# roatienza/efficientspeech

Hardware: AMD Instinct MI355X
Metric: mel-frames/sec (whole node), full Phoneme2Mel forward (higher is better)
Workload: dtype f32 (weight GEMMs: fp32 operands split into 2 f16 pieces (22 significand bits, weights pre-scaled 2^8), 3 f16-MFMA products, fp32 accumulate)

## Files before the change

efficientspeech_amd/csrc/chain16.h:

```cpp
#pragma once
#include "esmi_dev.h"
#include "wave_chain.h"

namespace esmi {
namespace c16 {

typedef unsigned u32x2 __attribute__((ext_vector_type(2)));

__device__ __forceinline__ float row_sum4(float v) {
    v += swap16_f(v);
    v += swap32_f(v);
    return v;
}
__device__ __forceinline__ float row_max4(float v) {
    v = fmaxf(v, swap16_f(v));
    v = fmaxf(v, swap32_f(v));
    return v;
}

__device__ __forceinline__ f32x4 mma(const u32x4& w1, const u32x4& w2, const f16x2p& a, f32x4 c) {
    c = mfma16_f16(w1, a.h2, c);
    c = mfma16_f16(w2, a.h1, c);
    c = mfma16_f16(w1, a.h1, c);
    return c;
// ... 17 lines not shown
    }
}

template <int N>
struct WFrags { u32x4 w1[N], w2[N]; };
template <int NT16, int NTW, int N>
__device__ __forceinline__ void wfrags_load(WFrags<N>& f, int at, const float* W0, int lw, int G) {
#pragma unroll
    for (int nt = 0; nt < NT16; ++nt) {
        const float* wp = W0 + ((4 * G) * NTW + (nt >> 1)) * 256 + 64 * (nt & 1) + lw;
        f.w1[at + nt] = *reinterpret_cast<const u32x4*>(wp);
        f.w2[at + nt] = *reinterpret_cast<const u32x4*>(wp + NTW * 256);
    }
}
template <int N>
__device__ __forceinline__ void mma_all(f32x4 (&acc)[N], const WFrags<N>& f, const f16x2p& a) {
#pragma unroll
    for (int n = 0; n < N; ++n) acc[n] = mfma16_f16(f.w1[n], a.h2, acc[n]);
#pragma unroll
    for (int n = 0; n < N; ++n) acc[n] = mfma16_f16(f.w2[n], a.h1, acc[n]);
#pragma unroll
    for (int n = 0; n < N; ++n) acc[n] = mfma16_f16(f.w1[n], a.h1, acc[n]);
}
template <int NT16, int NTW, int KS, typename BOp>
__device__ __forceinline__ void gemm_pf(f32x4 (&acc)[NT16], const float* W0, int lw, int G0, BOp bop) {
    WFrags<NT16> f[KS];
#pragma unroll
    for (int ks = 0; ks < KS; ++ks) wfrags_load<NT16, NTW, NT16>(f[ks], 0, W0, lw, G0 + ks);
    sched_fence();
#pragma unroll
    for (int ks = 0; ks < KS; ++ks) mma_all<NT16>(acc, f[ks], bop(ks));
}

__device__ __forceinline__ f16x2p planes_load(const unsigned* rowp, int ks, int chalf) {
    f16x2p a;
    a.h1 = *reinterpret_cast<const u32x4*>(rowp + 16 * ks);
    a.h2 = *reinterpret_cast<const u32x4*>(rowp + 16 * ks + chalf);
    return a;
}
__device__ __forceinline__ int wpos(int lane) { const int g = lane >> 4; return 4 * (g & 1) + 2 * (g >> 1); }
__device__ __forceinline__ void planes_store(unsigned* rowp, int nt, int chalf, const f32x4& v) {
    unsigned h1a, h2a, h1b, h2b;
    split_f16_pair(v[0], v[1], h1a, h2a);
    split_f16_pair(v[2], v[3], h1b, h2b);
    *reinterpret_cast<u32x2*>(rowp + 8 * nt) = u32x2{h1a, h1b};
    *reinterpret_cast<u32x2*>(rowp + 8 * nt + chalf) = u32x2{h2a, h2b};
}
__device__ __forceinline__ unsigned gl_lane(int lane) { const int g = lane >> 4; return (unsigned)((16 * (g >> 1) + 4 * (g & 1)) * 4); }
__device__ __forceinline__ f16x2p global_bop(BufRsrc r, unsigned off, int ks) {
    const f32x4 x0 = buf_ld4(r, off + 128u * ks), x1 = buf_ld4(r, off + 128u * ks + 32u);
    return split_f16x2(x0, x1);
}

template <int NT16>
__device__ __forceinline__ void layernorm(f32x4 (&v)[NT16], const f32x4 (&g)[NT16], const f32x4 (&b)[NT16], float eps = 1e-5f) {
    const float inv_c = 1.0f / (float)(16 * NT16);
    float s = 0.0f;
#pragma unroll
    for (int nt = 0; nt < NT16; ++nt) s += (v[nt][0] + v[nt][1]) + (v[nt][2] + v[nt][3]);
    const float mean = row_sum4(s) * inv_c;
    float q = 0.0f;
#pragma unroll
    for (int nt = 0; nt < NT16; ++nt) {
#pragma unroll
        for (int e = 0; e < 4; ++e) {
            v[nt][e] -= mean;
            q = fmaf(v[nt][e], v[nt][e], q);
        }
    }
    const float rstd = rsqrt_fast_f32(row_sum4(q) * inv_c + eps);
#pragma unroll
    for (int nt = 0; nt < NT16; ++nt) {
#pragma unroll
        for (int e = 0; e < 4; ++e) v[nt][e] = fmaf(v[nt][e] * rstd, g[nt][e], b[nt][e]);
    }
}

__device__ __forceinline__ void dma_frags(const float* gsrc, float* ldst, int nfrag, int w, int nw, int lane, int rot = 0) {
    rot %= nfrag;
    for (int f = w; f < nfrag; f += nw) {
        int fr = f + rot;
        fr = fr >= nfrag ? fr - nfrag : fr;
        lds_dma16(gsrc + fr * 256 + 4 * lane, ldst + fr * 256, lane);
    }
}

__device__ __forceinline__ f32x4 ld4_lds(const float* p) { return *reinterpret_cast<const f32x4*>(p); }
__device__ __forceinline__ f32x4 fmaf4(const f32x4& v, float s, const f32x4& b) {
    f32x4 o;
#pragma unroll
    for (int e = 0; e < 4; ++e) o[e] = fmaf(v[e], s, b[e]);
    return o;
}
__device__ __forceinline__ f32x4 relu4(const f32x4& v) {
    f32x4 o;
#pragma unroll
    for (int e = 0; e < 4; ++e) o[e] = fmaxf(v[e], 0.0f);
    return o;
}

}
}
```

efficientspeech_amd/csrc/enc_block16.h:

```cpp
#pragma once
#include "chain16.h"
#include "enc_attn_ffn.h"

namespace esmi {

struct B016Lds {
    static constexpr int C = 32, LD = C + 4, NK = 128, LDX = NK + 4;
    static constexpr int xP = 0;
    static constexpr int xT = xP + 128 * LD;
    static constexpr int y1P = xT + C * LDX;
    static constexpr int priv = y1P + 130 * LD;
    static constexpr int priv_sz = 2 * 16 * LD;
    static constexpr int par = priv + 8 * priv_sz;
    static constexpr int wts = par + 512;
    static constexpr int total = wts + 24 * 256;
};
static_assert(B016Lds::total * 4 <= 160 * 1024, "enc_b0_16: LDS");
enum { B0_PROJB = 0, B0_LN1G = 32, B0_LN1B = 64, B0_FFNB = 96, B0_FFNB0 = 128, B0_FFNB2 = 160, B0_MLP2B = 192, B0_LN2G = 224, B0_LN2B = 256 };

template <int NKT>
__device__ __forceinline__ void enc_b0_16_body(const EncAttnFfnP& p) {
    using namespace c16;
    typedef B016Lds M;
    constexpr int C = M::C, LD = M::LD, LDX = M::LDX;
    ESMI_DYN_LDS(lds);
    ESMI_CT_INIT(0);
    ESMI_CT();
    const int nw = (int)(blockDim.x >> 6), w = uniform_i(wave_id());
    const int lane = lane_id(), i = lane & 15, g = lane >> 4;
    const int b = (int)blockIdx.x, rot = b;
    const int pos = 16 * w + i;
    unsigned* const ldu = reinterpret_cast<unsigned*>(lds);
    unsigned* const xP = ldu + M::xP;
    unsigned* const xT = ldu + M::xT;
    unsigned* const y1P = ldu + M::y1P;
    float* const xf = lds + M::priv + w * M::priv_sz;
    unsigned* const qP = ldu + M::priv + w * M::priv_sz + 16 * LD;
    float* const par = lds + M::par;
    float* const wM = lds + M::wts, * const wO = wM + 4 * 256, * const wF = wO + 4 * 256, * const w2 = wF + 12 * 256;
    const int wp = wpos(lane), lw1 = wlane(lane, 1);
    const f32x4 z4 = zero4();
    const int* idb = p.m.ids + (long)b * p.m.n_in;
    int id[3];
#pragma unroll
    for (int j = 0; j < 3; ++j) {
        const int ti = pos + j - 1;
        const bool ok = ti >= 0 && ti < p.m.n_in;
        const int v = idb[ok ? ti : 0];
        id[j] = !ok ? -1 : ((v < 0 || v >= p.m.vocab) ? 0 : v);
    }
    dma_frags(p.m.qkv_w, wM, 4, w, nw, lane, rot);
    dma_frags(p.proj_w, wO, 4, w, nw, lane, rot);
    dma_frags(p.ffn_w, wF, 12, w, nw, lane, rot);
    dma_frags(p.mlp2_w, w2, 4, w, nw, lane, rot);
    {
        const int v8 = lane >> 3, c8 = 4 * (lane & 7);
        auto pick8 = [&](const float* a0, const float* a1, const float* a2, const float* a3, const float* a4, const float* a5, const float* a6,
                         const float* a7) __attribute__((always_inline)) {
            const float* lo = v8 & 1 ? (v8 & 2 ? a3 : a1) : (v8 & 2 ? a2 : a0);
            const float* hi = v8 & 1 ? (v8 & 2 ? a7 : a5) : (v8 & 2 ? a6 : a4);
            return (v8 & 4 ? hi : lo) + c8;
        };
        if (w == 0 % nw) lds_dma16(pick8(p.proj_b, p.ln1_g, p.ln1_b, p.ffn_b, p.ffn_b0, p.ffn_b2, p.mlp2_b, p.ln2_g), par, lane);
        if (w == 1 % nw) lds_dma16(p.ln2_b + c8, par + B0_LN2B, lane);
    }
    if (w == 0 && lane < LD) {
        y1P[lane] = 0u;
        y1P[(16 * nw + 1) * LD + lane] = 0u;
    }
    if (nw < NKT) {
        for (int e = (int)threadIdx.x; e < C * LDX; e += (int)blockDim.x) xT[e] = 0u;
        for (int e = (int)threadIdx.x + 16 * nw * LD; e < 16 * NKT * LD; e += (int)blockDim.x) xP[e] = 0u;
        wg_sync_lds();
    }
// ... 125 lines not shown
        for (int nt = 0; nt < 2; ++nt) {
            const f32x4 pb = ld4_lds(par + B0_PROJB + 16 * nt + 4 * g);
            gg[nt] = ld4_lds(par + B0_LN1G + 16 * nt + 4 * g);
            bb[nt] = ld4_lds(par + B0_LN1B + 16 * nt + 4 * g);
            y[nt] = fmaf4(y[nt], kF16WScaleInv, pb) + xacc[nt];
        }
        layernorm<2>(y, gg, bb);
#pragma unroll
        for (int nt = 0; nt < 2; ++nt) {
            if (rz || rout) y[nt] = z4;
            planes_store(y1P + (1 + pos) * LD + wp, nt, C / 2, y[nt]);
        }
    }
    ESMI_CT();
    wg_sync_lds();
    ESMI_CT();
    {
        f32x4 m[2] = {z4, z4};
        WFrags<2> ff[3];
        f16x2p fa[3];
#pragma unroll
        for (int j = 0; j < 3; ++j) {
            fa[j] = planes_load(y1P + (pos + j) * LD + 4 * g, 0, C / 2);
            wfrags_load<2, 1, 2>(ff[j], 0, wF + 4 * j * 256, lw1, 0);
        }
        sched_fence();
#pragma unroll
        for (int j = 0; j < 3; ++j) mma_all<2>(m, ff[j], fa[j]);
#pragma unroll
        for (int nt = 0; nt < 2; ++nt) {
            const f32x4 cb = ld4_lds(par + B0_FFNB + 16 * nt + 4 * g), cb0 = ld4_lds(par + B0_FFNB0 + 16 * nt + 4 * g),
                        cb2 = ld4_lds(par + B0_FFNB2 + 16 * nt + 4 * g);
            f32x4 v;
#pragma unroll
            for (int e = 0; e < 4; ++e) {
                const float bias = cb[e] - (pos == 0 ? cb0[e] : 0.0f) - (pos == p.N - 1 ? cb2[e] : 0.0f);
                v[e] = gelu_fast_f32(fmaf(m[nt][e], kF16WScaleInv, bias));
            }
            planes_store(qP + i * LD + wp, nt, C / 2, v);
        }
        lds_wave_sync();
        f32x4 z[2] = {z4, z4};
        const unsigned* rowp = qP + i * LD + 4 * g;
        gemm_pf<2, 1, 1>(z, w2, lw1, 0, [&](int) __attribute__((always_inline)) { return planes_load(rowp, 0, C / 2); });
        f32x4 gg[2], bb[2];
#pragma unroll
        for (int nt = 0; nt < 2; ++nt) {
            const f32x4 b2 = ld4_lds(par + B0_MLP2B + 16 * nt + 4 * g);
            gg[nt] = ld4_lds(par + B0_LN2G + 16 * nt + 4 * g);
            bb[nt] = ld4_lds(par + B0_LN2B + 16 * nt + 4 * g);
            z[nt] = fmaf4(z[nt], kF16WScaleInv, b2) + y[nt];
        }
        layernorm<2>(z, gg, bb);
        const BufRsrc r_out = make_rsrc(p.out + (long)b * p.N * C, (long)p.N * C * 4);
        const unsigned off = rout ? kBufOOB : (unsigned)(pos * C * 4);
#pragma unroll
        for (int nt = 0; nt < 2; ++nt) buf_st4(r_out, off + (unsigned)((16 * nt + 4 * g) * 4), rz ? z4 : z[nt]);
    }
    ESMI_CT();
}

template <int NKT>
__global__ __launch_bounds__(64 * 8, 2) void enc_b0_16_kernel(const EncAttnFfnP p) {
    enc_b0_16_body<NKT>(p);
}

struct B116Lds {
    static constexpr int C = 64, LD = C + 4, CIN = 32, NK = 64, LDX = NK + 4, LDC = 2 * C + 4;
    static constexpr int r1 = 0;
    static constexpr int r2 = r1 + 66 * LD;
    static constexpr int r3 = r2 + 64 * LD;
    static constexpr int r3_sz = 8 * 16 * LD;
    static constexpr int stats = r3 + r3_sz;
    static constexpr int par = stats + 256;
    static constexpr int wY = par + 768;
    static constexpr int wX = wY + 48 * 256;
    static constexpr int total = wX + 32 * 256;
};
static_assert(64 * B116Lds::LDC <= B116Lds::r3_sz && B116Lds::total * 4 <= 160 * 1024, "enc_b1_16: LDS");
enum { B1_PROJB = 0, B1_LN1G = 64, B1_LN1B = 128, B1_FFNB = 192, B1_FFNB0 = 256, B1_FFNB2 = 320, B1_MLP2B = 384, B1_LN2G = 448, B1_LN2B = 512 };

__device__ __forceinline__ void layernorm_pair16(f32x4 (&v)[2], const f32x4 (&gg)[2], const f32x4 (&bb)[2], float* st, int c, int i, int g,
                                                 float eps = 1e-5f) {
    using namespace c16;
    float s = (v[0][0] + v[0][1]) + (v[0][2] + v[0][3]) + ((v[1][0] + v[1][1]) + (v[1][2] + v[1][3]));
    const float mean_l = row_sum4(s) * (1.0f / 32.0f);
    float q = 0.0f;
#pragma unroll
    for (int nt = 0; nt < 2; ++nt) {
#pragma unroll
        for (int e = 0; e < 4; ++e) {
            const float d = v[nt][e] - mean_l;
            q = fmaf(d, d, q);
        }
    }
    const float m2_l = row_sum4(q);
    if (g == 0) *reinterpret_cast<f32x2*>(st + (c * 16 + i) * 2) = f32x2{mean_l, m2_l};
    wg_sync_lds();
    const f32x2 o = *reinterpret_cast<const f32x2*>(st + ((c ^ 1) * 16 + i) * 2);
    const float ma = c == 0 ? mean_l : o[0], mb = c == 0 ? o[0] : mean_l;
    const float qa = c == 0 ? m2_l : o[1], qb = c == 0 ? o[1] : m2_l;
    const float mean = 0.5f * (ma + mb);
    const float d = mb - ma;
    const float m2 = (qa + qb) + d * d * 16.0f;
    const float rstd = rsqrt_fast_f32(m2 * (1.0f / 64.0f) + eps);
#pragma unroll
    for (int nt = 0; nt < 2; ++nt) {
#pragma unroll
        for (int e = 0; e < 4; ++e) v[nt][e] = fmaf((v[nt][e] - mean) * rstd, gg[nt][e], bb[nt][e]);
    }
}

__device__ __forceinline__ void enc_b1_16_body(const EncAttnFfnP& p) {
    using namespace c16;
    typedef B116Lds M;
    constexpr int C = M::C, LD = M::LD, LDX = M::LDX, LDC = M::LDC, CIN = M::CIN, NKT = 4;
    ESMI_DYN_LDS(lds);
    ESMI_CT_INIT(1);
    ESMI_CT();
    const int nw = (int)(blockDim.x >> 6), w = uniform_i(wave_id());
    const int nrt = nw >> 1, rt = w >> 1, c = w & 1;
    const int lane = lane_id(), i = lane & 15, g = lane >> 4;
    const int b = (int)blockIdx.x, rot = b;
    const int pos = 16 * rt + i;
    unsigned* const ldu = reinterpret_cast<unsigned*>(lds);
    unsigned* const xP = ldu + M::r1;
    unsigned* const y1P = ldu + M::r1;
    unsigned* const xT = ldu + M::r2;
    unsigned* const hidP = ldu + M::r2;
    float* const xf = lds + M::r3 + w * (16 * LD);
    unsigned* const qP = ldu + M::r3 + w * (16 * LD);
    unsigned* const ctxP = ldu + M::r3;
    float* const st = lds + M::stats + rt * 64;
    float* const par = lds + M::par;
    float* const wY = lds + M::wY, * const wX = lds + M::wX;
    const int wp = wpos(lane), lw2 = wlane(lane, 2), lw4 = wlane(lane, 4);
    const f32x4 z4 = zero4();
    const bool rout = pos >= p.N;
    const BufRsrc r_in = make_rsrc(p.m.x_in + (long)b * p.m.n_in * CIN, (long)p.m.n_in * CIN * 4);
    const f16x2p a_in = global_bop(r_in, rout ? kBufOOB : (unsigned)(2 * pos * CIN * 4) + gl_lane(lane), 0);
    dma_frags(p.m.merge_w, wY, 8, w, nw, lane, rot);
    dma_frags(p.m.qkv_w, wY + 8 * 256, 32, w, nw, lane, rot);
    dma_frags(p.proj_w, wX, 32, w, nw, lane, rot);
    {
        const int v4 = lane >> 4, c4 = 4 * (lane & 15);
        auto pick4 = [&](const float* a0, const float* a1, const float* a2, const float* a3) __attribute__((always_inline)) {
            return (v4 & 2 ? (v4 & 1 ? a3 : a2) : (v4 & 1 ? a1 : a0)) + c4;
        };
        if (w == 0 % nw) lds_dma16(pick4(p.proj_b, p.ln1_g, p.ln1_b, p.ffn_b), par, lane);
        if (w == 1 % nw) lds_dma16(pick4(p.ffn_b0, p.ffn_b2, p.mlp2_b, p.ln2_g), par + 256, lane);
        if (w == 2 % nw) lds_dma16(p.ln2_b + c4, par + 512, lane);
    }
    if (nrt < NKT) {
        for (int e = (int)threadIdx.x; e < C * LDX; e += (int)blockDim.x) xT[e] = 0u;
        for (int e = (int)threadIdx.x + 16 * nrt * LD; e < 16 * NKT * LD; e += (int)blockDim.x) xP[e] = 0u;
        wg_sync_lds();
    }
    unsigned mb = 0;
    {
        const BufRsrc r_mask = make_rsrc(p.mask ? p.mask + (long)b * p.mask_len : nullptr, p.mask_len);
        for (int q = 0; q < p.mask_pool; ++q) {
            const int idx = pos * p.mask_pool + q;
            mb |= buf_ld_u8(r_mask, (unsigned)idx) | (unsigned)(p.mask && idx >= p.mask_len);
        }
    }
    const bool rz = !rout && mb != 0;
    wait_vm0();
    wg_sync_lds();
    ESMI_CT();
    f32x4 xh[2] = {z4, z4};
    gemm_pf<2, 2, 1>(xh, wY + c * 256, lw2, 0, [&](int) __attribute__((always_inline)) { return a_in; });
#pragma unroll
    for (int nt = 0; nt < 2; ++nt) {
        xh[nt] = rout ? z4 : xh[nt] * kF16WScaleInv;
        planes_store(xP + pos * LD + wp, 2 * c + nt, C / 2, xh[nt]);
        *reinterpret_cast<f32x4*>(xf + i * (CIN + 4) + 16 * nt + 4 * g) = xh[nt];
    }
    lds_wave_sync();
#pragma unroll
    for (int ct = 0; ct < 2; ++ct) {
        f32x4 v;
#pragma unroll
        for (int r = 0; r < 4; ++r) v[r] = xf[(4 * g + r) * (CIN + 4) + 16 * ct + i];
        unsigned h1a, h2a, h1b, h2b;
        split_f16_pair(v[0], v[1], h1a, h2a);
        split_f16_pair(v[2], v[3], h1b, h2b);
        unsigned* dst = xT + (32 * c + 16 * ct + i) * LDX + 16 * (rt >> 1) + 4 * g + 2 * (rt & 1);
        *reinterpret_cast<u32x2*>(dst) = u32x2{h1a, h1b};
        *reinterpret_cast<u32x2*>(dst + M::NK / 2) = u32x2{h2a, h2b};
    }
    wg_sync_lds();
    ESMI_CT();
    {
// ... 97 lines not shown
        for (int nt = 0; nt < 2; ++nt) {
            const int col = 32 * c + 16 * nt + 4 * g;
            gg[nt] = ld4_lds(par + B1_LN1G + col);
            bb[nt] = ld4_lds(par + B1_LN1B + col);
            y[nt] = fmaf4(y[nt], kF16WScaleInv, ld4_lds(par + B1_PROJB + col)) + xh[nt];
        }
        layernorm_pair16(y, gg, bb, st, c, i, g);
    }
    dma_frags(p.mlp2_w, wX, 16, w, nw, lane, rot);
#pragma unroll
    for (int nt = 0; nt < 2; ++nt) {
        if (rz || rout) y[nt] = z4;
        planes_store(y1P + (1 + pos) * LD + wp, 2 * c + nt, C / 2, y[nt]);
    }
    wait_vm0();
    wg_sync_lds();
    ESMI_CT();
    {
        f32x4 m[2] = {z4, z4};
#pragma unroll
        for (int j = 0; j < 3; ++j) {
            const unsigned* rowp = y1P + (pos + j) * LD + 4 * g;
            gemm_pf<2, 2, 2>(m, wY + j * 16 * 256 + c * 256, lw2, 0, [&](int ks) __attribute__((always_inline)) { return planes_load(rowp, ks, C / 2); });
        }
#pragma unroll
        for (int nt = 0; nt < 2; ++nt) {
            const int col = 32 * c + 16 * nt + 4 * g;
            const f32x4 cb = ld4_lds(par + B1_FFNB + col), cb0 = ld4_lds(par + B1_FFNB0 + col), cb2 = ld4_lds(par + B1_FFNB2 + col);
            f32x4 v;
#pragma unroll
            for (int e = 0; e < 4; ++e) {
                const float bias = cb[e] - (pos == 0 ? cb0[e] : 0.0f) - (pos == p.N - 1 ? cb2[e] : 0.0f);
                v[e] = gelu_fast_f32(fmaf(m[nt][e], kF16WScaleInv, bias));
            }
            planes_store(hidP + pos * LD + wp, 2 * c + nt, C / 2, v);
        }
    }
    wait_vm0();
    wg_sync_lds();
    ESMI_CT();
    {
        f32x4 z[2] = {z4, z4};
        const unsigned* rowp = hidP + pos * LD + 4 * g;
        gemm_pf<2, 2, 2>(z, wX + c * 256, lw2, 0, [&](int ks) __attribute__((always_inline)) { return planes_load(rowp, ks, C / 2); });
        f32x4 gg[2], bb[2];
#pragma unroll
        for (int nt = 0; nt < 2; ++nt) {
            const int col = 32 * c + 16 * nt + 4 * g;
            gg[nt] = ld4_lds(par + B1_LN2G + col);
            bb[nt] = ld4_lds(par + B1_LN2B + col);
            z[nt] = fmaf4(z[nt], kF16WScaleInv, ld4_lds(par + B1_MLP2B + col)) + y[nt];
        }
        layernorm_pair16(z, gg, bb, st, c, i, g);
        const BufRsrc r_out = make_rsrc(p.out + (long)b * p.N * C, (long)p.N * C * 4);
        const unsigned off = rout ? kBufOOB : (unsigned)(pos * C * 4);
#pragma unroll
        for (int nt = 0; nt < 2; ++nt) buf_st4(r_out, off + (unsigned)((32 * c + 16 * nt + 4 * g) * 4), rz ? z4 : z[nt]);
    }
    ESMI_CT();
}

__global__ __launch_bounds__(64 * 8, 2) void enc_b1_16_kernel(const EncAttnFfnP p) {
    enc_b1_16_body(p);
}

}
```

efficientspeech_amd/csrc/enc_va16.h:

```cpp
#pragma once
#include "chain16.h"
#include "enc_fuse_va.h"
#include "va_decide.h"

namespace esmi {

constexpr int kVa16MaxWaves = 8;
constexpr int kVa16Dim = 32;

struct Va16Lds {
    static constexpr int DIM = kVa16Dim;
    static constexpr int LDD = DIM + 4, LDT = 3 * DIM + 4, LDC = 2 * DIM + 4;
    static constexpr int ROWS = 16 * kVa16MaxWaves + 2;
    static constexpr int fused = 0;
    static constexpr int region = fused + ROWS * LDD;
    static constexpr int priv = 16 * LDC + 17 * LDD;
    static constexpr int region_sz = (ROWS * LDT > kVa16MaxWaves * priv ? ROWS * LDT : kVa16MaxWaves * priv);
    static constexpr int sdur = region + region_sz;
    static constexpr int par = sdur + 128;
    static constexpr int par_sz = 32 * 32 + 4 * 128;
    static constexpr int emb = par + par_sz;
    static constexpr int wA = emb + 2 * DIM * DIM;
    static constexpr int half = 9 * 1024;
    static constexpr int wB = wA + half;
    static constexpr int total = wB + half;
};
static_assert(Va16Lds::total * 4 <= 160 * 1024, "enc_va16: LDS");
inline int va16_lds_bytes() { return Va16Lds::total * (int)sizeof(float); }

enum { PV_MLPB0 = 0, PV_MLPB1 = 32, PV_UPB1 = 64, PV_FUSEB = 96, PV_LN2G = 128, PV_LN2B = 160, PV_EDGE = 192 ,
       PV_PRED = 256 ,
       PV_HEADB = 1024, PV_HEADG = PV_HEADB + 128, PV_HEADBE = PV_HEADG + 128 };

template <int KU>
__device__ __forceinline__ void enc_va16_body(const FuseVaP& p) {
    using namespace c16;
    typedef Va16Lds M;
    constexpr int DIM = M::DIM, LDD = M::LDD, LDT = M::LDT, LDC = M::LDC;
    static_assert((20 + 4 * KU) * 256 <= Va16Lds::half, "enc_va16: Fuse weights exceed an LDS half");
    ESMI_DYN_LDS(lds);
    ESMI_CT_INIT(2);
    ESMI_CT();
    const int nw = (int)(blockDim.x >> 6), w = uniform_i(wave_id());
    const int lane = lane_id(), i = lane & 15, g = lane >> 4;
    const int b = (int)blockIdx.x;
    const int r0 = 16 * w, pos = r0 + i;
    unsigned* const ldu = reinterpret_cast<unsigned*>(lds);
    unsigned* const fusedT = ldu + M::fused;
    unsigned* const hidT = ldu + M::region;
    unsigned* const catP = ldu + M::region + w * M::priv;
    unsigned* const tmpP = catP + 16 * LDC;
    int* const sdur = reinterpret_cast<int*>(lds + M::sdur);
    float* const par = lds + M::par;
    float* const embT = lds + M::emb;
    float* const wA = lds + M::wA;
    float* const wB = lds + M::wB;
    const int wp = wpos(lane);
    const int lw1 = wlane(lane, 1), lw4 = wlane(lane, 4);
    const f32x4 z4 = zero4();
    const int rot = (int)blockIdx.x;

    const bool rout = pos >= p.T;
    const BufRsrc r_mask = make_rsrc(p.mask ? p.mask + (long)b * p.T : nullptr, p.T);
    const bool rz = !rout && buf_ld_u8(r_mask, (unsigned)pos) != 0;
    const BufRsrc r_feat = make_rsrc(p.feat ? p.feat + (long)b * p.T * 4 * DIM : nullptr, (long)p.T * 4 * DIM * 4);
    const unsigned frow = rout ? kBufOOB : (unsigned)(pos * 4 * DIM * 4);
    const BufRsrc r_pt = make_rsrc(p.pitch_t ? p.pitch_t + (long)b * p.T : nullptr, (long)p.T * 4);
    const BufRsrc r_et = make_rsrc(p.energy_t ? p.energy_t + (long)b * p.T : nullptr, (long)p.T * 4);
    const BufRsrc r_dt = make_rsrc(p.dur_t ? p.dur_t + (long)b * p.T : nullptr, (long)p.T * 4);
    const unsigned trow = rout ? kBufOOB : (unsigned)(pos * 4);
    const float tv_p = buf_ld(r_pt, trow), tv_e = buf_ld(r_et, trow), tv_d = buf_ld(r_dt, trow);
    const float lb0 = p.pred[0].lin_b[0], lb1 = p.pred[1].lin_b[0], lb2 = p.pred[2].lin_b[0];
    const float sc_p = ctl_scale(p.pitch_s, b), sc_e = ctl_scale(p.energy_s, b), sc_d = ctl_scale(p.dur_s, b);
    const int e_i = (lane & 31) < DIM - 1 ? (lane & 31) : DIM - 2;
    const float edge_p = p.pred[0].bins[e_i], edge_e = p.pred[1].bins[e_i];
    const int n1 = p.n_i[1];
    const int n_base = floor_div(r0 - (KU - 1), 2);
    const int n_i = n_base + i;
    const BufRsrc r_f0 = make_rsrc(p.feats[0] + (long)b * p.n_i[0] * DIM, (long)p.n_i[0] * DIM * 4);
    const BufRsrc r_f1 = make_rsrc(p.feats[1] + (long)b * n1 * 2 * DIM, (long)n1 * 2 * DIM * 4);
    const unsigned o0 = rout ? kBufOOB : (unsigned)(pos * DIM * 4) + gl_lane(lane);
    const unsigned o1 = (n_i < 0 || n_i >= n1) ? kBufOOB : (unsigned)(n_i * 2 * DIM * 4) + gl_lane(lane);
    const f32x4 g0a = buf_ld4(r_f0, o0), g0b = buf_ld4(r_f0, o0 + 32u);
    const f32x4 g1a = buf_ld4(r_f1, o1), g1b = buf_ld4(r_f1, o1 + 32u), g1c = buf_ld4(r_f1, o1 + 128u), g1d = buf_ld4(r_f1, o1 + 160u);
    {
        dma_frags(p.mlp_w[0], wA, 4, w, nw, lane, rot);
        dma_frags(p.mlp_w[1], wA + 4 * 256, 8, w, nw, lane, rot);
        dma_frags(p.up_w[1], wA + 12 * 256, 4 * KU, w, nw, lane, rot);
        dma_frags(p.fuse_w, wA + (12 + 4 * KU) * 256, 8, w, nw, lane, rot);
        ESMI_CT();
        const int v8 = lane >> 3, c8 = 4 * (lane & 7);
        auto pick8 = [&](const float* a0, const float* a1, const float* a2, const float* a3, const float* a4, const float* a5, const float* a6,
                         const float* a7) __attribute__((always_inline)) {
            const float* lo = v8 & 1 ? (v8 & 2 ? a3 : a1) : (v8 & 2 ? a2 : a0);
            const float* hi = v8 & 1 ? (v8 & 2 ? a7 : a5) : (v8 & 2 ? a6 : a4);
            return (v8 & 4 ? hi : lo) + c8;
        };
        if (w == 0 % nw) lds_dma16(pick8(p.mlp_b[0], p.mlp_b[1], p.up_b[1], p.fuse_b, p.pred[2].ln2_g, p.pred[2].ln2_b, p.fuse_b, p.fuse_b), par, lane);
#pragma unroll
        for (int q = 0; q < 3; ++q) {
            const PredW& d = p.pred[q];
            if (w == (1 + q) % nw) lds_dma16(pick8(d.conv1_b, d.ln1_g, d.ln1_b, d.conv2_b, d.lin_w, d.lin_w, d.lin_w, d.lin_w), par + PV_PRED + 256 * q, lane);
        }
        if (p.h0) {
            if (w == 4 % nw) lds_dma16((lane < 32 ? p.head_b : p.head_g) + 4 * (lane & 31), par + PV_HEADB, lane);
            if (w == 5 % nw) lds_dma16(p.head_beta + 4 * (lane & 31), par + PV_HEADBE, lane);
        }
        if (w == 0) {
            if (lane < LDD) {
                fusedT[lane] = 0u;
                fusedT[(16 * nw + 1) * LDD + lane] = 0u;
            }
        }
        if (lane < LDD) tmpP[16 * LDD + lane] = 0u;
    }
    ESMI_CT();
    wait_vm0();
    ESMI_CT();
    wg_sync_lds();
    ESMI_CT();
    const f16x2p a0 = split_f16x2(g0a, g0b), a10 = split_f16x2(g1a, g1b), a11 = split_f16x2(g1c, g1d);
#pragma unroll
    for (int q = 0; q < 3; ++q) dma_frags(p.pred[q].conv1_w, wB + q * 12 * 256, 12, w, nw, lane, rot);
    dma_frags(p.pred[0].emb, embT, 4, w, nw, lane, rot);
    dma_frags(p.pred[1].emb, embT + DIM * DIM, 4, w, nw, lane, rot);
    if (w == 0) {
        const int l5 = lane & 31;
        par[PV_EDGE + lane] = l5 < DIM - 1 ? (lane < 32 ? edge_p : edge_e) : INFINITY;
    }
    f32x4 acc[2];
    {
        acc[0] = z4; acc[1] = z4;
        gemm_pf<2, 1, 1>(acc, wA, lw1, 0, [&](int) __attribute__((always_inline)) { return a0; });
#pragma unroll
        for (int nt = 0; nt < 2; ++nt) {
            const f32x4 bc = ld4_lds(par + PV_MLPB0 + 16 * nt + 4 * g);
            planes_store(catP + i * LDC + wp, nt, LDC / 2 - 2, fmaf4(acc[nt], kF16WScaleInv, bc));
        }
    }
    {
        acc[0] = z4; acc[1] = z4;
        gemm_pf<2, 1, 2>(acc, wA + 4 * 256, lw1, 0, [&](int ks) __attribute__((always_inline)) { return ks ? a11 : a10; });
        const bool n_ok = n_i >= 0 && n_i < n1;
#pragma unroll
        for (int nt = 0; nt < 2; ++nt) {
            const f32x4 bc = ld4_lds(par + PV_MLPB1 + 16 * nt + 4 * g);
            planes_store(tmpP + i * LDD + wp, nt, DIM / 2, n_ok ? fmaf4(acc[nt], kF16WScaleInv, bc) : z4);
        }
        lds_wave_sync();
        acc[0] = z4; acc[1] = z4;
        WFrags<2> uf[KU];
        f16x2p ua[KU];
#pragma unroll
        for (int j = 0; j < KU; ++j) {
            const int q = pos - j, nq = q >> 1;
            const bool ok = q >= 0 && (q & 1) == 0 && nq < n1;
            ua[j] = planes_load(tmpP + (ok ? nq - n_base : 16) * LDD + 4 * g, 0, DIM / 2);
            wfrags_load<2, 1, 2>(uf[j], 0, wA + (12 + 4 * j) * 256, lw1, 0);
        }
        sched_fence();
#pragma unroll
        for (int j = 0; j < KU; ++j) mma_all<2>(acc, uf[j], ua[j]);
#pragma unroll
        for (int nt = 0; nt < 2; ++nt) {
            const f32x4 bc = ld4_lds(par + PV_UPB1 + 16 * nt + 4 * g);
            planes_store(catP + i * LDC + wp, 2 + nt, LDC / 2 - 2, fmaf4(acc[nt], kF16WScaleInv, bc));
        }
        lds_wave_sync();
    }
    f32x4 fz[2];
    {
        acc[0] = z4; acc[1] = z4;
        const unsigned* rowp = catP + i * LDC + 4 * g;
        gemm_pf<2, 1, 2>(acc, wA + (12 + 4 * KU) * 256, lw1, 0, [&](int ks) __attribute__((always_inline)) { return planes_load(rowp, ks, LDC / 2 - 2); });
// ... 237 lines not shown
```

efficientspeech_amd/csrc/tu_enc_block16.hip:

```cpp
#include "launch.h"
#include "enc_block16.h"
#include "enc_va16.h"

using namespace esmi;
ESMI_TU_RANGE_SETTER(enc_block16)
ESMI_TU_CHAIN_TRACE_SETTER(enc_block16)

namespace esmi {

static bool b16_common_ok(const EncAttnFfnP& p) { return p.fold && p.N >= 1 && p.m.qkv_w && p.proj_w && p.ffn_w && p.mlp2_w; }
static bool b0_16_ok(const EncAttnFfnP& p) {
    return b16_common_ok(p) && p.C == 32 && p.h == 1 && p.m.k == 3 && p.m.stride == 1 && p.m.ids && p.m.emb_conv && p.N <= 128 && p.m.n_in == p.N;
}
static bool b1_16_ok(const EncAttnFfnP& p, int c_in) {
    return b16_common_ok(p) && p.C == 64 && p.h == 2 && p.m.k == 1 && p.m.stride == 2 && c_in == 32 && p.m.x_in && !p.m.ids && p.N <= 64 &&
           p.m.n_in >= 2 * p.N - 1;
}

#if ESMI_CHAIN_SPLIT
struct EncAll16P { EncAttnFfnP b0, b1; FuseVaP va; };
template <int NKT>
__global__ __launch_bounds__(64 * 8, 2) void enc_all16_kernel(const EncAll16P p) {
    enc_b0_16_body<NKT>(p.b0);
    wait_vm0();
    __syncthreads();
    enc_b1_16_body(p.b1);
    wait_vm0();
    __syncthreads();
    enc_va16_body<3>(p.va);
}
#endif

int launch_enc_all16(const EncAttnFfnP& b0, const EncAttnFfnP& b1, int c_in1, const FuseVaP& va, int dim, int kernel, hipStream_t st) {
#if ESMI_CHAIN_SPLIT
    if (!b0_16_ok(b0) || !b1_16_ok(b1, c_in1) || !enc_va16_ok(va, dim, kernel)) return ESMI_ERR_UNSUPPORTED;
    if (va.T != b0.N || b0.B != b1.B || b0.B != va.B) return ESMI_ERR_UNSUPPORTED;
    int nw = (b0.N + 15) / 16;
    const int nw1 = 2 * ((b1.N + 15) / 16);
    nw = (nw > nw1 ? nw : nw1);
    nw += nw & 1;
    if (nw > 8) return ESMI_ERR_UNSUPPORTED;
    EncAll16P q;
    q.b0 = b0; q.b1 = b1; q.va = va;
    int lds = B016Lds::total > B116Lds::total ? B016Lds::total : B116Lds::total;
    lds = (lds > Va16Lds::total ? lds : Va16Lds::total) * (int)sizeof(float);
#define ESMI_ALL(NKT) { ESMI_LAUNCH_LDS((enc_all16_kernel<NKT>), dim3(b0.B), dim3(64 * nw), lds, st, q); return launch_status(); }
    if (nw <= 2) ESMI_ALL(2)
    if (nw <= 4) ESMI_ALL(4)
    ESMI_ALL(8)
#undef ESMI_ALL
#else
    (void)b0; (void)b1; (void)c_in1; (void)va; (void)dim; (void)kernel; (void)st;
    return ESMI_ERR_UNSUPPORTED;
#endif
}

int launch_enc_block16(const EncAttnFfnP& p, int expansion, int c_in, hipStream_t st) {
#if ESMI_CHAIN_SPLIT
    if (expansion != 1) return ESMI_ERR_UNSUPPORTED;
    EncAttnFfnP q = p;
    q.wgs_per_b = 1; q.halo = 0;
    if (b0_16_ok(p)) {
        const int nw = (p.N + 15) / 16, lds = B016Lds::total * (int)sizeof(float);
#define ESMI_B0(NKT) { ESMI_LAUNCH_LDS((enc_b0_16_kernel<NKT>), dim3(p.B), dim3(64 * nw), lds, st, q); return launch_status(); }
        if (nw <= 2) ESMI_B0(2)
        if (nw <= 4) ESMI_B0(4)
        ESMI_B0(8)
#undef ESMI_B0
    }
    if (b1_16_ok(p, c_in)) {
        const int nrt = (p.N + 15) / 16, lds = B116Lds::total * (int)sizeof(float);
        ESMI_LAUNCH_LDS(enc_b1_16_kernel, dim3(p.B), dim3(128 * nrt), lds, st, q);
        return launch_status();
    }
    return ESMI_ERR_UNSUPPORTED;
#else
    (void)p; (void)expansion; (void)c_in; (void)st;
    return ESMI_ERR_UNSUPPORTED;
#endif
}

}
```

efficientspeech_amd/csrc/wavesim_shim.h:

```cpp
#pragma once

#ifdef ESMI_WAVESIM
#include "wavesim.h"
#define ESMI_DYN_LDS(name) float* name = (float*)wavesim::dyn_lds()
#define ESMI_LAUNCH(kern, grid, block, lds, stream, ...) \
    wavesim::launch(#kern, grid, block, lds, [&]() { kern(__VA_ARGS__); })
#else
#include <hip/hip_runtime.h>
#define ESMI_DYN_LDS(name) extern __shared__ __attribute__((aligned(16))) float name[]
#define ESMI_LAUNCH(kern, grid, block, lds, stream, ...) hipLaunchKernelGGL(kern, grid, block, lds, stream, __VA_ARGS__)
#endif

#include "esmi_types.h"

#ifndef ESMI_CHAIN_SPLIT
#define ESMI_CHAIN_SPLIT 1
#endif

namespace esmi {

#ifdef ESMI_WAVESIM
constexpr const char* kBackendName = "wavesim";
constexpr int kReduceGroups = 4;
constexpr int kLossBlocks = 8;
// ... 261 lines not shown
#else
    return __builtin_amdgcn_exp2f(x * 1.4426950408889634f);
#endif
}
__device__ __forceinline__ float rsqrt_fast_f32(float x) {
#ifdef ESMI_WAVESIM
    return 1.0f / sqrtf(x);
#else
    return __builtin_amdgcn_rsqf(x);
#endif
}
__device__ __forceinline__ float rcp_fast_f32(float x) {
#ifdef ESMI_WAVESIM
    return 1.0f / x;
#else
    return __builtin_amdgcn_rcpf(x);
#endif
}
__device__ __forceinline__ long long clock_shader() {
#ifdef ESMI_WAVESIM
    return 0;
#else
    return (long long)__builtin_amdgcn_s_memtime();
#endif
}
__device__ __forceinline__ long long clock_real100() {
#ifdef ESMI_WAVESIM
    return 0;
#else
    return (long long)__builtin_amdgcn_s_memrealtime();
#endif
}
__device__ __forceinline__ int opaque_i(int v) {
#ifndef ESMI_WAVESIM
    asm volatile("" : "+v"(v));
#endif
    return v;
}
__device__ __forceinline__ int uniform_i(int v) {
#ifdef ESMI_WAVESIM
    return v;
#else
    return __builtin_amdgcn_readfirstlane(v);
#endif
}
__device__ __forceinline__ float ctl_scale(const float* scale, int b) {
#ifdef ESMI_WAVESIM
    return scale ? scale[b] : 1.0f;
#else
    typedef const __attribute__((address_space(4))) float* const_f32_ptr;
    return scale ? *(const_f32_ptr)(scale + uniform_i(b)) : 1.0f;
#endif
}
__device__ __forceinline__ void lds_dma16(const void* gsrc_lane, void* lds_wave_base, int lane) {
#ifdef ESMI_WAVESIM
    reinterpret_cast<f32x4*>(lds_wave_base)[lane] = *reinterpret_cast<const f32x4*>(gsrc_lane);
#else
    (void)lane;
    __builtin_amdgcn_global_load_lds((const __attribute__((address_space(1))) void*)gsrc_lane,
                                     (__attribute__((address_space(3))) void*)lds_wave_base, 16, 0, 0);
#endif
}
constexpr unsigned kBufOOB = 0x80000000u;
#ifdef ESMI_WAVESIM
struct BufRsrc { const char* base; unsigned bytes; };
__device__ __forceinline__ BufRsrc make_rsrc(const void* p, long bytes) {
    BufRsrc r = {static_cast<const char*>(p), p ? (unsigned)(bytes < 0 ? 0 : (bytes > 0x7fffffffL ? 0x7fffffffL : bytes)) : 0u};
    return r;
}
__device__ __forceinline__ float buf_ld(const BufRsrc& r, unsigned off) {
    return (off < r.bytes && off + 4u <= r.bytes) ? *reinterpret_cast<const float*>(r.base + off) : 0.0f;
}
__device__ __forceinline__ f32x4 buf_ld4(const BufRsrc& r, unsigned off) {
    f32x4 z = {0.f, 0.f, 0.f, 0.f};
    return (off < r.bytes && off + 16u <= r.bytes) ? *reinterpret_cast<const f32x4*>(r.base + off) : z;
}
__device__ __forceinline__ unsigned buf_ld_u8(const BufRsrc& r, unsigned off) {
    return off < r.bytes ? (unsigned)*reinterpret_cast<const unsigned char*>(r.base + off) : 0u;
}
__device__ __forceinline__ f32x4 buf_ld4s(const BufRsrc& r, unsigned voff, unsigned soff) { return buf_ld4(r, voff + soff); }
__device__ __forceinline__ void buf_st(const BufRsrc& r, unsigned off, float v) {
    if (off < r.bytes && off + 4u <= r.bytes) *reinterpret_cast<float*>(const_cast<char*>(r.base) + off) = v;
}
__device__ __forceinline__ void buf_st_i(const BufRsrc& r, unsigned off, int v) {
    if (off < r.bytes && off + 4u <= r.bytes) *reinterpret_cast<int*>(const_cast<char*>(r.base) + off) = v;
}
__device__ __forceinline__ void buf_st_s(const BufRsrc& r, unsigned voff, unsigned soff, float v) { buf_st(r, voff == kBufOOB ? kBufOOB : voff + soff, v); }
__device__ __forceinline__ void buf_st4(const BufRsrc& r, unsigned off, const f32x4& v) {
    if (off < r.bytes && off + 16u <= r.bytes) *reinterpret_cast<f32x4*>(const_cast<char*>(r.base) + off) = v;
}
__device__ __forceinline__ void lds_wave_sync() { wavesim::shfl_i(0, 0); }
__device__ __forceinline__ void wait_vm0() {}
__device__ __forceinline__ void wg_sync_lds() { __syncthreads(); }
#else
typedef __amdgpu_buffer_rsrc_t BufRsrc;
__device__ __forceinline__ BufRsrc make_rsrc(const void* p, long bytes) {
    const int n = p ? (int)(bytes < 0 ? 0 : (bytes > 0x7fffffffL ? 0x7fffffffL : bytes)) : 0;
    return __builtin_amdgcn_make_buffer_rsrc(const_cast<void*>(p), 0, n, 0x00020000);
}
__device__ __forceinline__ float buf_ld(BufRsrc r, unsigned off) {
    return __builtin_bit_cast(float, __builtin_amdgcn_raw_buffer_load_b32(r, (int)off, 0, 0));
}
__device__ __forceinline__ f32x4 buf_ld4(BufRsrc r, unsigned off) {
    return __builtin_bit_cast(f32x4, __builtin_amdgcn_raw_buffer_load_b128(r, (int)off, 0, 0));
}
__device__ __forceinline__ unsigned buf_ld_u8(BufRsrc r, unsigned off) {
// ... 70 lines not shown
```

Measured before the change: 882.4 million.

## Carry encoder block outputs through LDS in fused encoder kernel

In the fused encoder kernel, block 0 and block 1 outputs now stay in LDS as split f16 planes instead of being written to global memory and read back by the next stage. Block 0's output is also held in registers for the variance-adaptor stage. A kernarg prefetch touch is added and the full vm-wait/syncthreads pairs are replaced by LDS-only barriers. This removes the global round trips and the split work between stages, at the cost of LDS-offset aliasing constraints and fallback conditions when the buffers do not chain.

```diff
diff --git a/efficientspeech_amd/csrc/chain16.h b/efficientspeech_amd/csrc/chain16.h
--- a/efficientspeech_amd/csrc/chain16.h
+++ b/efficientspeech_amd/csrc/chain16.h
@@ -93,6 +93,12 @@
     return split_f16x2(x0, x1);
 }
 
+struct Carry16 {
+    static constexpr int ld0 = 32 + 4, ld1 = 64 + 4;
+    static constexpr int x0 = 0, x0_end = x0 + 128 * ld0;
+    static constexpr int x1 = 31208, x1_end = x1 + 64 * ld1;
+};
+
 template <int NT16>
 __device__ __forceinline__ void layernorm(f32x4 (&v)[NT16], const f32x4 (&g)[NT16], const f32x4 (&b)[NT16], float eps = 1e-5f) {
     const float inv_c = 1.0f / (float)(16 * NT16);
diff --git a/efficientspeech_amd/csrc/enc_block16.h b/efficientspeech_amd/csrc/enc_block16.h
--- a/efficientspeech_amd/csrc/enc_block16.h
+++ b/efficientspeech_amd/csrc/enc_block16.h
@@ -16,10 +16,11 @@
     static constexpr int total = wts + 24 * 256;
 };
 static_assert(B016Lds::total * 4 <= 160 * 1024, "enc_b0_16: LDS");
+static_assert(c16::Carry16::x0 == B016Lds::xP && c16::Carry16::ld0 == B016Lds::LD && c16::Carry16::x0_end <= B016Lds::xT, "enc_all16: x0 carry");
 enum { B0_PROJB = 0, B0_LN1G = 32, B0_LN1B = 64, B0_FFNB = 96, B0_FFNB0 = 128, B0_FFNB2 = 160, B0_MLP2B = 192, B0_LN2G = 224, B0_LN2B = 256 };
 
-template <int NKT>
-__device__ __forceinline__ void enc_b0_16_body(const EncAttnFfnP& p) {
+template <int NKT, bool CARRY = false>
+__device__ __forceinline__ void enc_b0_16_body(const EncAttnFfnP& p, f16x2p* keep = nullptr) {
     using namespace c16;
     typedef B016Lds M;
     constexpr int C = M::C, LD = M::LD, LDX = M::LDX;
@@ -251,10 +252,18 @@
             z[nt] = fmaf4(z[nt], kF16WScaleInv, b2) + y[nt];
         }
         layernorm<2>(z, gg, bb);
-        const BufRsrc r_out = make_rsrc(p.out + (long)b * p.N * C, (long)p.N * C * 4);
-        const unsigned off = rout ? kBufOOB : (unsigned)(pos * C * 4);
-#pragma unroll
-        for (int nt = 0; nt < 2; ++nt) buf_st4(r_out, off + (unsigned)((16 * nt + 4 * g) * 4), rz ? z4 : z[nt]);
+        if constexpr (CARRY) {
+            unsigned* const x0c = ldu + Carry16::x0 + pos * Carry16::ld0;
+#pragma unroll
+            for (int nt = 0; nt < 2; ++nt) planes_store(x0c + wp, nt, C / 2, (rz || rout) ? z4 : z[nt]);
+            lds_wave_sync();
+            *keep = planes_load(x0c + 4 * g, 0, C / 2);
+        } else {
+            const BufRsrc r_out = make_rsrc(p.out + (long)b * p.N * C, (long)p.N * C * 4);
+            const unsigned off = rout ? kBufOOB : (unsigned)(pos * C * 4);
+#pragma unroll
+            for (int nt = 0; nt < 2; ++nt) buf_st4(r_out, off + (unsigned)((16 * nt + 4 * g) * 4), rz ? z4 : z[nt]);
+        }
     }
     ESMI_CT();
 }
@@ -277,6 +286,8 @@
     static constexpr int total = wX + 32 * 256;
 };
 static_assert(64 * B116Lds::LDC <= B116Lds::r3_sz && B116Lds::total * 4 <= 160 * 1024, "enc_b1_16: LDS");
+static_assert(c16::Carry16::x0_end <= B116Lds::stats, "enc_all16: x0 carry under block 1's entry DMA targets");
+static_assert(c16::Carry16::ld1 == B116Lds::LD && c16::Carry16::x1 >= B116Lds::wX && c16::Carry16::x1_end <= B116Lds::total, "enc_all16: x1 carry");
 enum { B1_PROJB = 0, B1_LN1G = 64, B1_LN1B = 128, B1_FFNB = 192, B1_FFNB0 = 256, B1_FFNB2 = 320, B1_MLP2B = 384, B1_LN2G = 448, B1_LN2B = 512 };
 
 __device__ __forceinline__ void layernorm_pair16(f32x4 (&v)[2], const f32x4 (&gg)[2], const f32x4 (&bb)[2], float* st, int c, int i, int g,
@@ -310,6 +321,7 @@
     }
 }
 
+template <bool CARRY = false>
 __device__ __forceinline__ void enc_b1_16_body(const EncAttnFfnP& p) {
     using namespace c16;
     typedef B116Lds M;
@@ -336,8 +348,17 @@
     const int wp = wpos(lane), lw2 = wlane(lane, 2), lw4 = wlane(lane, 4);
     const f32x4 z4 = zero4();
     const bool rout = pos >= p.N;
-    const BufRsrc r_in = make_rsrc(p.m.x_in + (long)b * p.m.n_in * CIN, (long)p.m.n_in * CIN * 4);
-    const f16x2p a_in = global_bop(r_in, rout ? kBufOOB : (unsigned)(2 * pos * CIN * 4) + gl_lane(lane), 0);
+    f16x2p a_in;
+    if constexpr (CARRY) {
+        const u32x4 zu = {0u, 0u, 0u, 0u};
+        a_in = planes_load(ldu + Carry16::x0 + (rout ? 0 : 2 * pos) * Carry16::ld0 + 4 * g, 0, CIN / 2);
+        a_in.h1 = rout ? zu : a_in.h1;
+        a_in.h2 = rout ? zu : a_in.h2;
+        if (nrt < NKT) wg_sync_lds();
+    } else {
+        const BufRsrc r_in = make_rsrc(p.m.x_in + (long)b * p.m.n_in * CIN, (long)p.m.n_in * CIN * 4);
+        a_in = global_bop(r_in, rout ? kBufOOB : (unsigned)(2 * pos * CIN * 4) + gl_lane(lane), 0);
+    }
     dma_frags(p.m.merge_w, wY, 8, w, nw, lane, rot);
     dma_frags(p.m.qkv_w, wY + 8 * 256, 32, w, nw, lane, rot);
     dma_frags(p.proj_w, wX, 32, w, nw, lane, rot);
@@ -541,16 +562,22 @@
             z[nt] = fmaf4(z[nt], kF16WScaleInv, ld4_lds(par + B1_MLP2B + col)) + y[nt];
         }
         layernorm_pair16(z, gg, bb, st, c, i, g);
-        const BufRsrc r_out = make_rsrc(p.out + (long)b * p.N * C, (long)p.N * C * 4);
-        const unsigned off = rout ? kBufOOB : (unsigned)(pos * C * 4);
-#pragma unroll
-        for (int nt = 0; nt < 2; ++nt) buf_st4(r_out, off + (unsigned)((32 * c + 16 * nt + 4 * g) * 4), rz ? z4 : z[nt]);
+        if constexpr (CARRY) {
+            unsigned* const x1c = ldu + Carry16::x1 + pos * Carry16::ld1;
+#pragma unroll
+            for (int nt = 0; nt < 2; ++nt) planes_store(x1c + wp, 2 * c + nt, C / 2, (rz || rout) ? z4 : z[nt]);
+        } else {
+            const BufRsrc r_out = make_rsrc(p.out + (long)b * p.N * C, (long)p.N * C * 4);
+            const unsigned off = rout ? kBufOOB : (unsigned)(pos * C * 4);
+#pragma unroll
+            for (int nt = 0; nt < 2; ++nt) buf_st4(r_out, off + (unsigned)((32 * c + 16 * nt + 4 * g) * 4), rz ? z4 : z[nt]);
+        }
     }
     ESMI_CT();
 }
 
 __global__ __launch_bounds__(64 * 8, 2) void enc_b1_16_kernel(const EncAttnFfnP p) {
-    enc_b1_16_body(p);
+    enc_b1_16_body<>(p);
 }
 
 }
diff --git a/efficientspeech_amd/csrc/enc_va16.h b/efficientspeech_amd/csrc/enc_va16.h
--- a/efficientspeech_amd/csrc/enc_va16.h
+++ b/efficientspeech_amd/csrc/enc_va16.h
@@ -26,14 +26,15 @@
     static constexpr int total = wB + half;
 };
 static_assert(Va16Lds::total * 4 <= 160 * 1024, "enc_va16: LDS");
+static_assert(c16::Carry16::x1 == Va16Lds::wB && c16::Carry16::x1_end <= Va16Lds::total, "enc_all16: x1 carry in weight half B");
 inline int va16_lds_bytes() { return Va16Lds::total * (int)sizeof(float); }
 
 enum { PV_MLPB0 = 0, PV_MLPB1 = 32, PV_UPB1 = 64, PV_FUSEB = 96, PV_LN2G = 128, PV_LN2B = 160, PV_EDGE = 192 ,
        PV_PRED = 256 ,
        PV_HEADB = 1024, PV_HEADG = PV_HEADB + 128, PV_HEADBE = PV_HEADG + 128 };
 
-template <int KU>
-__device__ __forceinline__ void enc_va16_body(const FuseVaP& p) {
+template <int KU, bool CARRY = false>
+__device__ __forceinline__ void enc_va16_body(const FuseVaP& p, const f16x2p* x0_keep = nullptr) {
     using namespace c16;
     typedef Va16Lds M;
     constexpr int DIM = M::DIM, LDD = M::LDD, LDT = M::LDT, LDC = M::LDC;
@@ -77,12 +78,25 @@
     const int n1 = p.n_i[1];
     const int n_base = floor_div(r0 - (KU - 1), 2);
     const int n_i = n_base + i;
-    const BufRsrc r_f0 = make_rsrc(p.feats[0] + (long)b * p.n_i[0] * DIM, (long)p.n_i[0] * DIM * 4);
-    const BufRsrc r_f1 = make_rsrc(p.feats[1] + (long)b * n1 * 2 * DIM, (long)n1 * 2 * DIM * 4);
-    const unsigned o0 = rout ? kBufOOB : (unsigned)(pos * DIM * 4) + gl_lane(lane);
-    const unsigned o1 = (n_i < 0 || n_i >= n1) ? kBufOOB : (unsigned)(n_i * 2 * DIM * 4) + gl_lane(lane);
-    const f32x4 g0a = buf_ld4(r_f0, o0), g0b = buf_ld4(r_f0, o0 + 32u);
-    const f32x4 g1a = buf_ld4(r_f1, o1), g1b = buf_ld4(r_f1, o1 + 32u), g1c = buf_ld4(r_f1, o1 + 128u), g1d = buf_ld4(r_f1, o1 + 160u);
+    f32x4 g0a, g0b, g1a, g1b, g1c, g1d;
+    f16x2p a0, a10, a11;
+    if constexpr (CARRY) {
+        const bool n_in = n_i >= 0 && n_i < n1;
+        const unsigned* rowp = ldu + Carry16::x1 + (n_in ? n_i : 0) * Carry16::ld1 + 4 * g;
+        const u32x4 zu = {0u, 0u, 0u, 0u};
+        a0 = *x0_keep;
+        a10 = planes_load(rowp, 0, DIM);
+        a11 = planes_load(rowp, 1, DIM);
+        a10.h1 = n_in ? a10.h1 : zu; a10.h2 = n_in ? a10.h2 : zu;
+        a11.h1 = n_in ? a11.h1 : zu; a11.h2 = n_in ? a11.h2 : zu;
+    } else {
+        const BufRsrc r_f0 = make_rsrc(p.feats[0] + (long)b * p.n_i[0] * DIM, (long)p.n_i[0] * DIM * 4);
+        const BufRsrc r_f1 = make_rsrc(p.feats[1] + (long)b * n1 * 2 * DIM, (long)n1 * 2 * DIM * 4);
+        const unsigned o0 = rout ? kBufOOB : (unsigned)(pos * DIM * 4) + gl_lane(lane);
+        const unsigned o1 = (n_i < 0 || n_i >= n1) ? kBufOOB : (unsigned)(n_i * 2 * DIM * 4) + gl_lane(lane);
+        g0a = buf_ld4(r_f0, o0); g0b = buf_ld4(r_f0, o0 + 32u);
+        g1a = buf_ld4(r_f1, o1); g1b = buf_ld4(r_f1, o1 + 32u); g1c = buf_ld4(r_f1, o1 + 128u); g1d = buf_ld4(r_f1, o1 + 160u);
+    }
     {
         dma_frags(p.mlp_w[0], wA, 4, w, nw, lane, rot);
         dma_frags(p.mlp_w[1], wA + 4 * 256, 8, w, nw, lane, rot);
@@ -119,7 +133,7 @@
     ESMI_CT();
     wg_sync_lds();
     ESMI_CT();
-    const f16x2p a0 = split_f16x2(g0a, g0b), a10 = split_f16x2(g1a, g1b), a11 = split_f16x2(g1c, g1d);
+    if constexpr (!CARRY) { a0 = split_f16x2(g0a, g0b); a10 = split_f16x2(g1a, g1b); a11 = split_f16x2(g1c, g1d); }
 #pragma unroll
     for (int q = 0; q < 3; ++q) dma_frags(p.pred[q].conv1_w, wB + q * 12 * 256, 12, w, nw, lane, rot);
     dma_frags(p.pred[0].emb, embT, 4, w, nw, lane, rot);
diff --git a/efficientspeech_amd/csrc/tu_enc_block16.hip b/efficientspeech_amd/csrc/tu_enc_block16.hip
--- a/efficientspeech_amd/csrc/tu_enc_block16.hip
+++ b/efficientspeech_amd/csrc/tu_enc_block16.hip
@@ -21,13 +21,18 @@
 struct EncAll16P { EncAttnFfnP b0, b1; FuseVaP va; };
 template <int NKT>
 __global__ __launch_bounds__(64 * 8, 2) void enc_all16_kernel(const EncAll16P p) {
-    enc_b0_16_body<NKT>(p.b0);
-    wait_vm0();
-    __syncthreads();
-    enc_b1_16_body(p.b1);
-    wait_vm0();
-    __syncthreads();
-    enc_va16_body<3>(p.va);
+    ESMI_CT_INIT(5);
+    kernarg_warm((int)sizeof(EncAttnFfnP), (int)(sizeof(EncAll16P) - sizeof(EncAttnFfnP)));
+    f16x2p x0_keep;
+    enc_b0_16_body<NKT, true>(p.b0, &x0_keep);
+    ESMI_CT();
+    wg_sync_lds();
+    ESMI_CT();
+    enc_b1_16_body<true>(p.b1);
+    ESMI_CT();
+    wg_sync_lds();
+    ESMI_CT();
+    enc_va16_body<3, true>(p.va, &x0_keep);
 }
 #endif
 
@@ -35,6 +40,9 @@
 #if ESMI_CHAIN_SPLIT
     if (!b0_16_ok(b0) || !b1_16_ok(b1, c_in1) || !enc_va16_ok(va, dim, kernel)) return ESMI_ERR_UNSUPPORTED;
     if (va.T != b0.N || b0.B != b1.B || b0.B != va.B) return ESMI_ERR_UNSUPPORTED;
+    if (b1.m.x_in != b0.out || b1.m.n_in != b0.N || va.depth != 2 || va.feats[0] != b0.out || va.n_i[0] != b0.N || va.feats[1] != b1.out ||
+        va.n_i[1] != b1.N)
+        return ESMI_ERR_UNSUPPORTED;
     int nw = (b0.N + 15) / 16;
     const int nw1 = 2 * ((b1.N + 15) / 16);
     nw = (nw > nw1 ? nw : nw1);
diff --git a/efficientspeech_amd/csrc/wavesim_shim.h b/efficientspeech_amd/csrc/wavesim_shim.h
--- a/efficientspeech_amd/csrc/wavesim_shim.h
+++ b/efficientspeech_amd/csrc/wavesim_shim.h
@@ -337,6 +337,18 @@
     return scale ? *(const_f32_ptr)(scale + uniform_i(b)) : 1.0f;
 #endif
 }
+__device__ __forceinline__ void kernarg_warm(int off, int bytes) {
+#ifdef ESMI_WAVESIM
+    (void)off; (void)bytes;
+#else
+    typedef const __attribute__((address_space(4))) int* const_i32_ptr;
+    const const_i32_ptr base = (const_i32_ptr)__builtin_amdgcn_kernarg_segment_ptr();
+    int acc = 0;
+#pragma unroll
+    for (int o = off; o < off + bytes; o += 64) acc |= base[o >> 2];
+    asm volatile("" :: "s"(acc));
+#endif
+}
 __device__ __forceinline__ void lds_dma16(const void* gsrc_lane, void* lds_wave_base, int lane) {
 #ifdef ESMI_WAVESIM
     reinterpret_cast<f32x4*>(lds_wave_base)[lane] = *reinterpret_cast<const f32x4*>(gsrc_lane);
```

Measured after the change: 884.2 million (median of 2 runs). No clear change (+0.2%).
